# tambetm/simple_dqn

Hardware: NVIDIA B200
Metric: DQN training steps/sec (batch 32, 84x84x4) (higher is better)
Workload: dtype f16x3-split (fp32 accumulate)

## Files before the change

### simple_dqn_b200/csrc/net.cu

```cuda
#include <stdlib.h>

#include <new>
#include <vector>

#include <cuda_fp16.h>

#include "net.cuh"
#include "net_umma.cuh"

namespace b200 {

struct HeadTrainArgs {
  int enable;
  const uint8_t* actions;
  const int64_t* rewards;
  const uint8_t* terminals;
  const int32_t* midx;
  double discount;
  int min_reward, max_reward;
  float clip;
  float* delta;
  const uint32_t* step;
  float* row_cost;
  float* dz4;
// ... 655 lines not shown
    B2_CHECK_CUDA(cudaEventRecord(ev[11], sB));
    B2_CHECK_CUDA(cudaEventRecord(ev[12], sC));
    B2_CHECK_CUDA(cudaStreamWaitEvent(st, ev[11], 0));
    B2_CHECK_CUDA(cudaStreamWaitEvent(st, ev[12], 0));
  }
  B2_CHECK_CUDA(cudaEventRecord(ev[4], sA));
  B2_CHECK_CUDA(cudaStreamWaitEvent(st, ev[4], 0));
  return B200DQN_OK;
}

static int backward_and_update(b200dqn_net* n, const FrameSource& fs, int rows, cudaStream_t st, bool update) {
  if (update && n->world > 1 && !g_prof_on && n->use_branches && st != nullptr &&
      n->cfg.math_mode == B200DQN_MATH_TCGEN05)
    return backward_and_update_multi(n, fs, rows, st);
  const bool branches = update && n->world == 1 && n->use_branches && (st != nullptr || g_prof_on);
  if (!branches) {
    for (int op = kFc1Wgrad; op <= kConv1Wgrad; ++op) B2_TRY(bwd_op(n, fs, rows, BwdOp(op), st));
    B2_TRY(cost_finish_on(n, rows, st));
    if (!update) return B200DQN_OK;
    if (n->world > 1) {
      B2_TRY(optimizer_range(n, 0, kLayers - 1, 1 | 2, rows, st, "grad_reduce"));
      B2_TRY(comm_allreduce_grads(n, st));
      B2_PROF("allreduce", st);
      B2_TRY(optimizer_range(n, 0, kLayers - 1, 4, rows, st, "optimizer"));
    } else {
      B2_TRY(optimizer_range(n, 0, kLayers - 1, 1 | 4, rows, st, "optimizer"));
    }
    return B200DQN_OK;
  }
  cudaStream_t sA = g_prof_on ? st : n->side[0], sB = g_prof_on ? st : n->side[1], sC = g_prof_on ? st : n->side[2];
  cudaStream_t sN = g_prof_on ? st : n->side[3];
  cudaEvent_t* ev = n->ev;
  const bool tc = n->cfg.math_mode == B200DQN_MATH_TCGEN05;
  static const bool fc1_fused_epilogue = getenv("B200DQN_FC1_FUSED") != nullptr;
  static const int nopdl_ops = getenv("B200DQN_NOPDL_OPS") ? int(strtol(getenv("B200DQN_NOPDL_OPS"), nullptr, 0)) : 0;
  if (getenv("B200DQN_WGRAD_ONE_STREAM") && !g_prof_on) sC = sB;
  auto chain_op = [&](BwdOp op) -> int {
    if (nopdl_ops >> int(op) & 1) {
      NoPdlScope plain;
      return bwd_op(n, fs, rows, op, st);
    }
    return bwd_op(n, fs, rows, op, st);
  };
  B2_CHECK_CUDA(cudaEventRecord(ev[0], st));
  B2_CHECK_CUDA(cudaStreamWaitEvent(sA, ev[0], 0));
  B2_CHECK_CUDA(cudaStreamWaitEvent(sN, ev[0], 0));
  {
    NoPdlScope side;
    if (!(tc && fc1_fused_epilogue)) B2_TRY(bwd_op(n, fs, rows, kFc1Wgrad, sA));
    B2_TRY(cost_finish_on(n, rows, sN));
    if (tc) B2_TRY(opt_fc2_small(n, rows, sN));
  }
  B2_TRY(chain_op(kFc1Dgrad));
  B2_CHECK_CUDA(cudaEventRecord(ev[1], st));
  static const char* fc1_when_env = getenv("B200DQN_OPT_FC1_WHEN");
  const int fc1_when = !fc1_when_env || g_prof_on ? 0 : !strcmp(fc1_when_env, "ev2") ? 2 : !strcmp(fc1_when_env, "ev3") ? 3
                       : !strcmp(fc1_when_env, "last") ? 4 : !strcmp(fc1_when_env, "skip") ? 5 : 0;
  auto opt_fc1_now = [&]() -> int {
    NoPdlScope side;
    if (tc && fc1_fused_epilogue) return umma_fc1_wgrad_fused(n, rows, sA, n->keep_grads);
    if (tc && n->defer_fc1) return fc1_update_deferred(n, sA);
    if (tc) return umma_opt_fc1(n, rows, sA);
    return optimizer_range(n, 3, 4, 1 | 4, rows, sA, "opt_fc");
  };
  B2_CHECK_CUDA(cudaStreamWaitEvent(sA, ev[1], 0));
  if (fc1_when == 0) B2_TRY(opt_fc1_now());
  B2_CHECK_CUDA(cudaStreamWaitEvent(sB, ev[1], 0));
  { NoPdlScope side; B2_TRY(bwd_op(n, fs, rows, kConv3Wgrad, sB)); }
  B2_TRY(chain_op(kConv3Dgrad));
  B2_CHECK_CUDA(cudaEventRecord(ev[2], st));
  if (fc1_when == 2) {
    B2_CHECK_CUDA(cudaStreamWaitEvent(sA, ev[2], 0));
    B2_TRY(opt_fc1_now());
  }
  B2_CHECK_CUDA(cudaStreamWaitEvent(sB, ev[2], 0));
  {
    NoPdlScope side;
    if (n->cfg.math_mode == B200DQN_MATH_TCGEN05) B2_TRY(umma_opt_conv(n, 2, rows, sB, "opt_conv3"));
    else B2_TRY(optimizer_range(n, 2, 2, 1 | 4, rows, sB, "opt_conv3"));
  }
  B2_CHECK_CUDA(cudaStreamWaitEvent(sC, ev[2], 0));
  { NoPdlScope side; B2_TRY(bwd_op(n, fs, rows, kConv2Wgrad, sC)); }
  B2_TRY(chain_op(kConv2Dgrad));
  B2_CHECK_CUDA(cudaEventRecord(ev[3], st));
  if (fc1_when == 3) {
    B2_CHECK_CUDA(cudaStreamWaitEvent(sA, ev[3], 0));
    B2_TRY(opt_fc1_now());
  }
  B2_CHECK_CUDA(cudaStreamWaitEvent(sC, ev[3], 0));
  {
    NoPdlScope side;
    if (n->cfg.math_mode == B200DQN_MATH_TCGEN05) B2_TRY(umma_opt_conv(n, 1, rows, sC, "opt_conv2"));
    else B2_TRY(optimizer_range(n, 1, 1, 1 | 4, rows, sC, "opt_conv2"));
  }
  B2_TRY(chain_op(kConv1Wgrad));
// ... 645 lines not shown

extern "C" int b200dqn_net_device_ptr(b200dqn_net* n, int which, void** dev_ptr, size_t* bytes) {
  B2_REQUIRE(n && dev_ptr, B200DQN_EINVAL, "net_device_ptr: null argument");
  void* p = nullptr;
  size_t b = 0;
  switch (which) {
    case B200DQN_NET_PTR_Q_ONLINE: p = n->d_q[0]; b = size_t(n->nb) * n->A * 4; break;
    case B200DQN_NET_PTR_Q_TARGET: p = n->d_q[1]; b = size_t(n->nb) * n->A * 4; break;
    case B200DQN_NET_PTR_DELTAS: p = n->d_delta; b = size_t(n->nb) * n->A * 4; break;
    case B200DQN_NET_PTR_GRADS: p = n->d_g; b = n->n_params * 4; break;
    case B200DQN_NET_PTR_WEIGHTS: p = n->d_w; b = n->n_params * 4; break;
    case B200DQN_NET_PTR_COST: p = n->d_cost; b = kCostRing * 4; break;
    case B200DQN_NET_PTR_H1: p = n->d_h1[0]; b = size_t(n->nb) * kP1 * kP1 * kC1 * 4; break;
    case B200DQN_NET_PTR_H2: p = n->d_h2[0]; b = size_t(n->nb) * kP2 * kP2 * kC2 * 4; break;
    case B200DQN_NET_PTR_H3: p = n->d_h3[0]; b = size_t(n->nb) * kFlat * 4; break;
    case B200DQN_NET_PTR_H4: p = n->d_h4[0]; b = size_t(n->nb) * kHidden * 4; break;
    default: B2_REQUIRE(false, B200DQN_EINVAL, "net_device_ptr: unknown selector %d", which);
  }
  *dev_ptr = p;
  if (bytes) *bytes = b;
  return B200DQN_OK;
}

extern "C" int b200dqn_net_set_keep_grads(b200dqn_net* n, int keep) {
  B2_REQUIRE(n, B200DQN_EINVAL, "null net");
  n->keep_grads = keep != 0;
  destroy_step_graphs(n);
  if (n->graph_train_exec) { cudaGraphExecDestroy(n->graph_train_exec); n->graph_train_exec = nullptr; }
  return B200DQN_OK;
}

extern "C" int b200dqn_net_get_grads(b200dqn_net* n, int layer, float* host_dW, void* stream) {
  B2_REQUIRE(n && host_dW && layer >= 0 && layer < kLayers, B200DQN_EINVAL, "net_get_grads: bad argument");
  B2_REQUIRE(n->cfg.math_mode != B200DQN_MATH_TCGEN05 || n->world > 1 || n->keep_grads ||
                 getenv("B200DQN_FC1_FUSED") == nullptr,
             B200DQN_ESTATE, "net_get_grads: call b200dqn_net_set_keep_grads(net, 1) before the step (fused optimizer)");
  DeviceGuard g(n->device);
  cudaStream_t st = as_stream(stream);
  const int64_t n4 = n->n_params / 4;
  if (n->world == 1) {
    k_optimizer<<<cdiv(n4, 256), 256, 0, st>>>(n->lt, n->d_part, n->d_g, n->d_w, n->d_s, 0, n4, 1 | 2, OptArgs{},
                                               KTrace{nullptr, 0});
    B2_LAUNCH_CHECK();
  } else if (n->xchg_ok && n->xchg_sched == 2 && n->d_xbuf && layer == 3) {
    const int64_t b4 = n->lt.off[3] / 4, e4 = n->lt.off[4] / 4;
    k_optimizer<<<cdiv(e4 - b4, 256), 256, 0, st>>>(n->lt, n->d_part, n->d_g, n->d_w, n->d_s, b4, e4, 1 | 2, OptArgs{},
                                                    KTrace{nullptr, 0});
    B2_LAUNCH_CHECK();
  }
  return xfer_params(n, n->d_g, layer, host_dW, false, st);
}

extern "C" int b200dqn_net_launches_per_step(const b200dqn_net* n, int* launches) {
  B2_REQUIRE(n && launches, B200DQN_EINVAL, "null argument");
  if (n->graph_def_launches > 0) {
    *launches = n->graph_def_launches;
  } else if (n->graph_launches > 0) {
    *launches = n->graph_launches;
  } else {
    const bool tc = n->cfg.math_mode == B200DQN_MATH_TCGEN05;
    *launches = 1 + 4 + 1 + 7 + (n->world > 1 ? (tc ? 7 : 2) : (tc ? 6 : 4));
  }
  return B200DQN_OK;
}
```

### simple_dqn_b200/csrc/net_umma.cu

```cuda
#include "net.cuh"
#include "net_umma.cuh"
#include "umma.cuh"
#include "umma2.cuh"
#include "umma_mn.cuh"
#include "conv1_tma.cuh"

namespace b200 {

__device__ __forceinline__ void ld8(const float* p, float v[8]) {
  const float4 a = *reinterpret_cast<const float4*>(p);
  const float4 b = *reinterpret_cast<const float4*>(p + 4);
  v[0] = a.x; v[1] = a.y; v[2] = a.z; v[3] = a.w; v[4] = b.x; v[5] = b.y; v[6] = b.z; v[7] = b.w;
}
__device__ __forceinline__ void st8(float* p, const float v[8]) {
  *reinterpret_cast<float4*>(p) = make_float4(v[0], v[1], v[2], v[3]);
  *reinterpret_cast<float4*>(p + 4) = make_float4(v[4], v[5], v[6], v[7]);
}
__device__ __forceinline__ void zero8(float v[8]) {
#pragma unroll
  for (int i = 0; i < 8; ++i) v[i] = 0.f;
}

struct UmmaState {
  __half* h16[3][2] = {};
  int64_t h_elems[3] = {};
  __half* dz16[4] = {};
  int64_t dz_elems[4] = {};
  uint8_t* img_fwd[2][4] = {};
  int64_t img_fwd_bytes[4] = {};
  uint8_t* im2col1 = nullptr;
  uint8_t* img_dgr[3] = {};
};
static inline UmmaState* ust(b200dqn_net* n) { return static_cast<UmmaState*>(n->umma_state); }

struct PlanePair {
  __half* hi;
  int64_t lo_off;
};
// ... 187 lines not shown
    return {(int64_t(n * P + yy) * P + xx) * KO, yy, xx, ok};
  }
  __device__ bool a_chunk(int, const umma2::RowCtx& rc, int kk, int64_t& off) const {
    const int rp = kk / (RT * KO), sp = (kk / KO) % RT, ko = kk % KO;
    const int p = rc.y - rp, q = rc.x - sp;
    off = rc.base - (rp * P + sp) * KO + ko;
    return p >= 0 && p < P && q >= 0 && q < P;
  }
  __device__ const uint8_t* b_tile(int z, int, int kb) const { return wimg + (int64_t(z) * (K / 64) + kb) * (C * 256); }
  __device__ void prefetch8(int z, int m, int c0, float pf[8]) const {
    const int n = m / (HC * HC), yx = m % (HC * HC), yy = yx / HC, xx = yx % HC;
    const int y = yy * ST + z / ST, xq = xx * ST + z % ST;
    if (y >= H || xq >= H) { zero8(pf); return; }
    ld8(x + (int64_t(n * H + y) * H + xq) * C + c0, pf);
  }
  __device__ void store8p(int z, int m, int c0, const float v[8], const float xv[8]) const {
    const int n = m / (HC * HC), yx = m % (HC * HC), yy = yx / HC, xx = yx % HC;
    const int y = yy * ST + z / ST, xq = xx * ST + z % ST;
    if (y >= H || xq >= H) return;
    const int64_t i = (int64_t(n * H + y) * H + xq) * C + c0;
    float o[8];
#pragma unroll
    for (int j = 0; j < 8; ++j) o[j] = xv[j] > 0.f ? v[j] : 0.f;
    if (dx) st8(dx + i, o);
    if (dx16.hi) umma2::split8_planes(o, dx16.hi + i, dx16.hi + dx16.lo_off + i);
  }
};

template <int H, int C, int R, int ST, int KO, int STG = 4>
struct WConvWgrad {
  static constexpr int P = (H - R) / ST + 1, KW = R * R * C;
  static_assert((R * C) % 64 == 0 && KO == 64, "64-element runs must not straddle a filter row");
  static constexpr int kBN = 64, kStages = STG;
  static constexpr bool kAExact = false, kARegs = false, kABulk = false, kFusedUpdate = false;
  PlanePair x16;
  PlanePair dz16;
  float* part;
  int rows, kb_per_split;
  __device__ int M(int) const { return KW; }
  __device__ int N(int) const { return KO; }
  __device__ void krange(int z, int& kb, int& ke) const {
    const int total = (rows * P * P + 63) / 64;
    kb = min(z * kb_per_split, total);
    ke = min(kb + kb_per_split, total);
  }
  __device__ umma_mn::PixCtx pix(int, int kpix) const {
    const int n = kpix / (P * P), pq = kpix % (P * P);
    return {n, pq / P, pq % P, kpix < rows * P * P};
  }
  __device__ umma2::Planes a_planes(int) const { return {x16.hi, x16.lo_off}; }
  __device__ bool a_run(int, const umma_mn::PixCtx& px, int mchunk, int64_t& off) const {
    const int m = mchunk * 64, r = m / (R * C), sc = m % (R * C);
    off = (int64_t(px.n * H + px.p * ST + r) * H + px.q * ST) * C + sc;
    return m < KW;
  }
  __device__ umma2::Planes b_planes(int) const { return {dz16.hi, dz16.lo_off}; }
  __device__ int64_t b_off(int, const umma_mn::PixCtx& px) const { return (int64_t(px.n * P + px.p) * P + px.q) * KO; }
  __device__ void store8(int z, int m, int n0, const float v[8]) const { st8(part + (int64_t(z) * KW + m) * KO + n0, v); }
};

struct WConv1Wgrad {
  static constexpr int kBN = 32, kStages = 4;
  static constexpr bool kAExact = true, kARegs = false, kABulk = true, kFusedUpdate = false;
  const uint8_t* im2col;
  PlanePair dz16;
  float* part;
  int rows, kb_per_split;
  int tile_rows;
  __device__ int M(int) const { return kK1; }
  __device__ int N(int) const { return kC1; }
  __device__ int total_kb() const {
    return tile_rows == 128 ? (rows * kP1 * kP1 + 63) / 64 : rows * conv1tma::kTilesPerSample * 2;
  }
  __device__ void krange(int z, int& kb, int& ke) const {
    const int total = total_kb();
    kb = min(z * kb_per_split, total);
    ke = min(kb + kb_per_split, total);
  }
  __device__ umma_mn::PixCtx pix(int, int kpix) const {
    if (tile_rows == 128) return {kpix, 0, 0, kpix < rows * kP1 * kP1};
    const int tile = kpix >> 7, local = kpix & 127;
    return {tile * tile_rows + local, 0, 0, local < tile_rows && tile < rows * conv1tma::kTilesPerSample};
  }
  __device__ const uint8_t* a_sub(int, int c, int kb) const {
    return im2col + (int64_t(kb >> 1) * (kK1 / 64) + c) * (128 * 128) + (kb & 1) * (64 * 128);
  }
  __device__ umma2::Planes b_planes(int) const { return {dz16.hi, dz16.lo_off}; }
  __device__ int64_t b_off(int, const umma_mn::PixCtx& px) const { return int64_t(px.n) * kC1; }
  __device__ void store8(int z, int m, int n0, const float v[8]) const {
    float o[8];
#pragma unroll
    for (int j = 0; j < 8; ++j) o[j] = v[j] * (1.0f / 255.0f);
    st8(part + (int64_t(z) * kK1 + m) * kC1 + n0, o);
  }
};

struct WFc1Wgrad {
  static constexpr int kBN = 64, kStages = 2;
  static constexpr bool kAExact = false, kARegs = false, kABulk = false, kFusedUpdate = false;
  PlanePair h3_16;
  PlanePair dz4_16;
  float* dw4;
  int rows;
  __device__ int M(int) const { return kFlat; }
  __device__ int N(int) const { return kHidden; }
  __device__ void krange(int, int& kb, int& ke) const { kb = 0; ke = (rows + 63) / 64; }
  __device__ umma_mn::PixCtx pix(int, int b) const { return {b, 0, 0, b < rows}; }
  __device__ umma2::Planes a_planes(int) const { return {h3_16.hi, h3_16.lo_off}; }
  __device__ bool a_run(int, const umma_mn::PixCtx& px, int mchunk, int64_t& off) const {
    off = int64_t(px.n) * kFlat + mchunk * 64;
    return mchunk * 64 < kFlat;
  }
  __device__ umma2::Planes b_planes(int) const { return {dz4_16.hi, dz4_16.lo_off}; }
  __device__ int64_t b_off(int, const umma_mn::PixCtx& px) const { return int64_t(px.n) * kHidden; }
  __device__ void store8(int, int m, int n0, const float v[8]) const { st8(dw4 + int64_t(m) * kHidden + n0, v); }
};

struct WFc1WgradGather {
  static constexpr int kBN = 64, kStages = 2;
  static constexpr bool kAExact = false, kARegs = false, kABulk = false, kFusedUpdate = false;
  const __half* h3g;
  const __half* dzg;
  int64_t h3_parity, h3_lo, dz_parity, dz_lo;
  const uint32_t* epoch;
  float* dw4;
  int rows;
  __device__ int M(int) const { return kFlat; }
  __device__ int N(int) const { return kHidden; }
  __device__ void krange(int, int& kb, int& ke) const { kb = 0; ke = (rows + 63) / 64; }
  __device__ umma_mn::PixCtx pix(int, int b) const { return {b, 0, 0, b < rows}; }
  __device__ umma2::Planes a_planes(int) const { return {h3g + int64_t(epoch[0] & 1) * h3_parity, h3_lo}; }
  __device__ bool a_run(int, const umma_mn::PixCtx& px, int mchunk, int64_t& off) const {
    off = int64_t(px.n) * kFlat + mchunk * 64;
    return mchunk * 64 < kFlat;
  }
  __device__ umma2::Planes b_planes(int) const { return {dzg + int64_t(epoch[1] & 1) * dz_parity, dz_lo}; }
  __device__ int64_t b_off(int, const umma_mn::PixCtx& px) const { return int64_t(px.n) * kHidden; }
  __device__ void store8(int, int m, int n0, const float v[8]) const { st8(dw4 + int64_t(m) * kHidden + n0, v); }
};

struct WFc1WgradFused {
  static constexpr int kBN = 64, kStages = 2;
  static constexpr bool kAExact = false, kARegs = false, kABulk = false, kFusedUpdate = true;
  PlanePair h3_16;
  PlanePair dz4_16;
  float* w;
  float* s;
  float* dw_out;
  uint8_t* img_dgr;
  int rows;
  OptArgs opt;
  __device__ int M(int) const { return kFlat; }
  __device__ int N(int) const { return kHidden; }
  __device__ void krange(int, int& kb, int& ke) const { kb = 0; ke = (rows + 63) / 64; }
  __device__ umma_mn::PixCtx pix(int, int b) const { return {b, 0, 0, b < rows}; }
  __device__ umma2::Planes a_planes(int) const { return {h3_16.hi, h3_16.lo_off}; }
  __device__ bool a_run(int, const umma_mn::PixCtx& px, int mchunk, int64_t& off) const {
    off = int64_t(px.n) * kFlat + mchunk * 64;
    return mchunk * 64 < kFlat;
  }
  __device__ umma2::Planes b_planes(int) const { return {dz4_16.hi, dz4_16.lo_off}; }
  __device__ int64_t b_off(int, const umma_mn::PixCtx& px) const { return int64_t(px.n) * kHidden; }
  __device__ void store8(int, int, int, const float*) const {}
  __device__ float step_scalar() const { return opt_step_scalar(opt); }
  __device__ void update8(int, int m, int n0, float l, const float g[8], float nw[8]) const {
    const int64_t i = int64_t(m) * kHidden + n0;
    if (dw_out) st8(dw_out + i, g);
    opt_update_vec<8>(opt, l, g, nw, w + i, s + i);
    uint4 hi, lo;
    umma::split8(nw, hi, lo);
    uint8_t* base = img_dgr + (int64_t(m / 128) * (kHidden / 64) + n0 / 64) * (128 * 256) +
                    umma::sw128_off(m % 128, (n0 % 64) / 8);
    *reinterpret_cast<uint4*>(base) = hi;
    *reinterpret_cast<uint4*>(base + 128 * 128) = lo;
  }
  __device__ void pack_col8(int, int, int, const float*) const {}
};

template <int K, int N>
struct PackFwdConv {
  static constexpr bool kRowMajorThreads = false;
  const float* w;
  __host__ __device__ int tiles() const { return 1; }
  __host__ __device__ int rows() const { return N; }
  __host__ __device__ int kblocks() const { return K / 64; }
  __device__ void src8(int, int r, int k0, float v[8]) const {
#pragma unroll
    for (int j = 0; j < 8; ++j) v[j] = w[(k0 + j) * N + r];
  }
};
struct PackFc1Dgrad {
  static constexpr bool kRowMajorThreads = true;
  const float* w;
  __host__ __device__ int tiles() const { return (kFlat + 127) / 128; }
  __host__ __device__ int rows() const { return 128; }
  __host__ __device__ int kblocks() const { return kHidden / 64; }
  __device__ void src8(int tile, int r, int k0, float v[8]) const {
    const int m = tile * 128 + r;
    if (m >= kFlat) { zero8(v); return; }
    ld8(w + m * kHidden + k0, v);
  }
};
template <int H, int C, int R, int ST, int KO>
struct PackConvDgrad {
  static constexpr int RT = R / ST, K = RT * RT * KO;
  static constexpr bool kRowMajorThreads = true;
  const float* w;
  __host__ __device__ int tiles() const { return ST * ST; }
  __host__ __device__ int rows() const { return C; }
// ... 477 lines not shown
      using P2 = WConvWgrad<kP1, kC1, 4, 2, kC2, 2>;
      if (shallow_ring(n, "conv2_wgrad")) {
        P2 p{PlanePair{u->h16[0][0], u->h_elems[0]}, PlanePair{u->dz16[2], u->dz_elems[2]},
             n->d_part + lt.part_off[1], rows, umma_wgrad_kb(1, rows)};
        return umma_mn::launch_umma_mn("conv2_wgrad", p, P::KW, kC2, lt.splits[1], st);
      }
      P p{PlanePair{u->h16[0][0], u->h_elems[0]}, PlanePair{u->dz16[2], u->dz_elems[2]},
          n->d_part + lt.part_off[1], rows, umma_wgrad_kb(1, rows)};
      return umma_mn::launch_umma_mn("conv2_wgrad", p, P::KW, kC2, lt.splits[1], st);
    }
    case 5: {
      UmmaState* u = ust(n);
      using P = V2ConvDgrad<kP1, kC1, 4, 2, kC2>;
      using P2 = V2ConvDgrad<kP1, kC1, 4, 2, kC2, 2>;
      if (shallow_ring(n, "conv2_dgrad")) {
        P2 p{PlanePair{u->dz16[2], u->dz_elems[2]}, u->img_dgr[2], n->d_h1[0], n->keep_grads ? n->d_dz1 : nullptr,
             PlanePair{u->dz16[3], u->dz_elems[3]}, rows};
        return umma2::launch_umma2("conv2_dgrad", p, rows * P::HC * P::HC, kC1, 4, st);
      }
      P p{PlanePair{u->dz16[2], u->dz_elems[2]}, u->img_dgr[2], n->d_h1[0], n->keep_grads ? n->d_dz1 : nullptr,
          PlanePair{u->dz16[3], u->dz_elems[3]}, rows};
      return umma2::launch_umma2("conv2_dgrad", p, rows * P::HC * P::HC, kC1, 4, st);
    }
    default: {
      UmmaState* u = ust(n);
      (void)src; (void)idx; (void)shift;
      WConv1Wgrad p{u->im2col1, PlanePair{u->dz16[3], u->dz_elems[3]}, n->d_part + lt.part_off[0], rows,
                    umma_wgrad_kb(0, rows), g_conv1_tma ? conv1tma::kTileRows : 128};
      return umma_mn::launch_umma_mn("conv1_wgrad", p, kK1, kC1, lt.splits[0], st);
    }
  }
}

int umma_fc1_wgrad_fused(b200dqn_net* n, int rows, cudaStream_t st, bool keep_grads) {
  UmmaState* u = ust(n);
  const LayerTable& lt = n->lt;
  WFc1WgradFused p{PlanePair{u->h16[2][0], u->h_elems[2]}, PlanePair{u->dz16[0], u->dz_elems[0]},
                   n->d_w + lt.off[3], n->d_s + lt.off[3], keep_grads ? n->d_part + lt.part_off[3] : nullptr,
                   u->img_dgr[0], rows, make_opt_args(n, rows)};
  return umma_mn::launch_umma_mn("fc1_wgrad+opt", p, kFlat, kHidden, 1, st);
}

int umma_fc1_splits(int rows) { return fc1_splits_for(rows); }
bool umma_has_backward() { return true; }
int umma_push_h3(b200dqn_net* n, cudaStream_t st) {
  UmmaState* u = ust(n);
  cudaStream_t sN = n->side[3];
  B2_CHECK_CUDA(cudaEventRecord(n->ev[13], st));
  B2_CHECK_CUDA(cudaStreamWaitEvent(sN, n->ev[13], 0));
  const int rc = comm_push_planes(n, 0, u->h16[2][0], u->h_elems[2], sN);
  if (rc) return rc;
  B2_CHECK_CUDA(cudaEventRecord(n->ev[14], sN));
  return B200DQN_OK;
}
int umma_push_dz4(b200dqn_net* n, cudaStream_t st) {
  UmmaState* u = ust(n);
  return comm_push_planes(n, 1, u->dz16[0], u->dz_elems[0], st);
}
int umma_gather_dz4_ll(b200dqn_net* n, cudaStream_t st) {
  UmmaState* u = ust(n);
  return comm_gather_dz4_ll(n, u->dz16[0], u->dz_elems[0], st, true);
}
int umma_fc1_wgrad_gathered(b200dqn_net* n, cudaStream_t st) {
  WFc1WgradGather p{reinterpret_cast<const __half*>(n->d_xbuf + n->x_h3_off),
                    reinterpret_cast<const __half*>(n->d_xbuf + n->x_dz_off),
                    n->x_h3_parity / 2, n->x_h3_lo, n->x_dz_parity / 2, n->x_dz_lo,
                    n->d_xpush_epoch, n->d_part + n->lt.part_off[3], n->nb * n->world};
  return umma_mn::launch_umma_mn("fc1_wgrad", p, kFlat, kHidden, 1, st);
}

int umma_forward_launches() { return 4; }
int umma_backward_launches() { return 7; }

// ... 7 lines not shown
```

### simple_dqn_b200/csrc/net_umma.cuh

```cuda
#pragma once
#include <cuda_fp16.h>

#include "common.cuh"
#include "comm_p2p.cuh"
#include "optim.cuh"

struct b200dqn_net;

namespace b200 {

OptArgs make_opt_args(const b200dqn_net* n, int rows);

int umma_net_init(b200dqn_net* n);
void umma_net_destroy(b200dqn_net* n);
int umma_weights_changed(b200dqn_net* n, cudaStream_t st);
int umma_target_synced(b200dqn_net* n, cudaStream_t st);
int umma_forward(b200dqn_net* n, const uint8_t* const src[2], const int32_t* const idx[2], const int shift[2],
                 const int64_t nframes[2], int nets, int rows, cudaStream_t st);
int umma_fc1_splits(int rows);
int umma_opt_fc1(b200dqn_net* n, int rows, cudaStream_t st, bool from_g = false, const uint32_t* gate = nullptr);
int umma_fc1_wgrad_fused(b200dqn_net* n, int rows, cudaStream_t st, bool keep_grads);
int umma_opt_conv(b200dqn_net* n, int l, int rows, cudaStream_t st, const char* label, bool from_g = false);
int umma_pack_layers(b200dqn_net* n, int which, int l0, int l1, cudaStream_t st);
void umma_dz4_planes(b200dqn_net* n, __half** hi, int64_t* lo_off);
int umma_wgrad_splits(int layer, int rows);
bool umma_has_backward();
int umma_backward_op(b200dqn_net* n, int op, const uint8_t* src, const int32_t* idx, int shift, int rows,
                     cudaStream_t st);
int umma_forward_launches();
int umma_backward_launches();

int comm_allreduce_grads(b200dqn_net* n, cudaStream_t st);
int comm_allreduce_range(b200dqn_net* n, int l0, int l1, cudaStream_t st);
int comm_xchg_range(b200dqn_net* n, int l0, int l1, int chan, cudaStream_t st, const char* label);
bool comm_gather_active(const b200dqn_net* n, cudaStream_t st);
int comm_xll_layer(b200dqn_net* n, int layer, cudaStream_t st, const char* label);
int comm_xll_args(b200dqn_net* n, int layer, XllArgs* out);
int umma_opt_conv_xll(b200dqn_net* n, int l, int rows, cudaStream_t st, const char* label);
int comm_push_planes(b200dqn_net* n, int chan, const void* hi, int64_t lo_off_elems, cudaStream_t st);
int comm_wait_pushes(b200dqn_net* n, cudaStream_t st, int dz_rows = 0);
bool comm_dz4_ll_enabled();
int comm_gather_dz4_ll(b200dqn_net* n, const void* hi, int64_t lo_off_elems, cudaStream_t st, bool wait_h3);
bool comm_head_push(const b200dqn_net* n, cudaStream_t st, HeadPush* out);
int umma_push_h3(b200dqn_net* n, cudaStream_t st);
int umma_push_dz4(b200dqn_net* n, cudaStream_t st);
int umma_gather_dz4_ll(b200dqn_net* n, cudaStream_t st);
int umma_fc1_wgrad_gathered(b200dqn_net* n, cudaStream_t st);
void comm_destroy(b200dqn_net* n);

}
```

### simple_dqn_b200/csrc/umma_mn.cuh

```cuda
#pragma once
#include "umma2.cuh"

namespace b200 {
namespace umma_mn {

using umma::kBM;
using umma2::kLoadThreads;
using umma2::kThreads2;
using umma2::Planes;

constexpr int kKB = 64;

using umma::make_desc_mn;
__host__ __device__ constexpr uint32_t make_idesc_f16_mn(int M, int N) {
  return (1u << 4) | (1u << 15) | (1u << 16) | (uint32_t(N >> 3) << 17) | (uint32_t(M >> 4) << 24);
}
__device__ __forceinline__ uint32_t mn_off(int kr, int j) {
  return uint32_t((kr >> 3) * 1024 + (kr & 7) * 128 + ((j ^ (kr & 7)) << 4));
}

struct PixCtx {
  int n, p, q;
  bool ok;
};
// ... 146 lines not shown
          umma2::cp_async16(dst + mn_off(kr, 4 + sub), src + bpl.lo_off + sub * 8, bytes);
        }
      }
      if constexpr (P::kARegs) fence_proxy_async_smem();
      umma2::cp_async_arrive_noinc(&s_full[s]);
    }

    pdl_launch_dependents();

    mbar_wait(&s_done, 0);
    umma::fence_after_sync();
    {
      const int q = warp & 3, half = warp >> 2;
      const int row = q * 32 + lane;
      const uint32_t lane_addr = tmem + (uint32_t(q * 32) << 16);
      constexpr int kColsPerHalf = BN / 2;
      constexpr int kChunks = kColsPerHalf / 8;
      constexpr int kPitch = BN * 4 + 16;
#pragma unroll
      for (int c = 0; c < kChunks; ++c) {
        const int col = half * kColsPerHalf + c * 8;
        float a0[8], a1[8];
        umma::tmem_ld8(lane_addr + col, a0);
        umma::tmem_ld8(lane_addr + BN + col, a1);
        umma::tmem_ld_wait();
#pragma unroll
        for (int j = 0; j < 8; ++j) a0[j] = fmaf(a1[j], umma::kLoInv, a0[j]);
        float* dst = reinterpret_cast<float*>(smem_gen + row * kPitch + col * 4);
        *reinterpret_cast<float4*>(dst) = make_float4(a0[0], a0[1], a0[2], a0[3]);
        *reinterpret_cast<float4*>(dst + 4) = make_float4(a0[4], a0[5], a0[6], a0[7]);
      }
      umma2::named_bar_sync(1, kLoadThreads);
      constexpr int kChunksPerRow = BN / 8;
      if constexpr (!P::kFusedUpdate) {
#pragma unroll
        for (int i = 0; i < kBM * kChunksPerRow / kLoadThreads; ++i) {
          const int id = tid + i * kLoadThreads;
          const int r = id / kChunksPerRow, cc = id % kChunksPerRow;
          const float* src = reinterpret_cast<const float*>(smem_gen + r * kPitch + cc * 32);
          const float4 v0 = *reinterpret_cast<const float4*>(src), v1 = *reinterpret_cast<const float4*>(src + 4);
          const float v[8] = {v0.x, v0.y, v0.z, v0.w, v1.x, v1.y, v1.z, v1.w};
          if (m0 + r < M && n0 + cc * 8 < N) p.store8(z, m0 + r, n0 + cc * 8, v);
        }
      } else {
        constexpr int kIt = kBM * kChunksPerRow / kLoadThreads;
        const float l_step = p.step_scalar();
#pragma unroll
        for (int i = 0; i < kIt; ++i) {
          const int id = tid + i * kLoadThreads;
          const int r = id / kChunksPerRow, cc = id % kChunksPerRow;
          float* src = reinterpret_cast<float*>(smem_gen + r * kPitch + cc * 32);
          const float4 v0 = *reinterpret_cast<const float4*>(src), v1 = *reinterpret_cast<const float4*>(src + 4);
          const float g[8] = {v0.x, v0.y, v0.z, v0.w, v1.x, v1.y, v1.z, v1.w};
          if (m0 + r < M && n0 + cc * 8 < N) {
            float nw[8];
            p.update8(z, m0 + r, n0 + cc * 8, l_step, g, nw);
            *reinterpret_cast<float4*>(src) = make_float4(nw[0], nw[1], nw[2], nw[3]);
            *reinterpret_cast<float4*>(src + 4) = make_float4(nw[4], nw[5], nw[6], nw[7]);
          }
        }
        umma2::named_bar_sync(1, kLoadThreads);
#pragma unroll
        for (int i = 0; i < (kBM / 8) * BN / kLoadThreads; ++i) {
          const int id = tid + i * kLoadThreads;
          const int nn = id % BN, mg = id / BN;
          if (m0 + mg * 8 < M && n0 + nn < N) {
            float wv[8];
#pragma unroll
            for (int j = 0; j < 8; ++j)
              wv[j] = *reinterpret_cast<const float*>(smem_gen + (mg * 8 + j) * kPitch + nn * 4);
            p.pack_col8(z, m0 + mg * 8, n0 + nn, wv);
          }
        }
      }
    }
  }
  umma::fence_before_sync();
  __syncthreads();
  if (warp == 8) {
    umma::fence_after_sync();
    umma::tmem_dealloc(tmem, C::kTmemCols);
  }
  kt_end(kt);
}

template <class P>
static int launch_umma_mn(const char* label, const P& p, int M, int N, int Z, cudaStream_t st) {
  using C = CfgMN<P>;
  static bool configured = false;
  if (!configured) {
    B2_CHECK_CUDA(cudaFuncSetAttribute(k_umma_mn<P>, cudaFuncAttributeMaxDynamicSharedMemorySize, C::kSmemBytes));
    configured = true;
  }
  dim3 grid((M + kBM - 1) / kBM, (N + C::BN - 1) / C::BN, Z);
  B2_CHECK_CUDA(launch_pdl(k_umma_mn<P>, grid, dim3(kThreads2), C::kSmemBytes, st, p, ktrace_slot(label)));
  B2_PROF(label, st);
  return B200DQN_OK;
}

}
}
```

Measured before the change: 13340.

## Add dedicated warp-specialized fc1 wgrad+Adam kernel with TMA weight/state streaming, enable by default

Adds a new persistent, warp-specialized kernel that computes the fc1 weight gradient with tcgen05 MMA into double-buffered TMEM accumulators. In the same kernel it applies the optimizer update, streaming weights and optimizer state through per-warp TMA load/store rings and writing the packed fp16 hi/lo swizzled image for the dgrad path. It becomes the default tc path whenever fc1 deferral is off, replacing the separate fc1 wgrad and fc1 optimizer launches and removing the old env-gated fused epilogue from the generic MN kernel. The aim is to cut one launch plus the round trip of the fp32 gradient through global memory, and to overlap MMA with the optimizer epilogue. The cost is a fixed CTA count (24 by default), host-side tensor-map encoding on every call, and more complex synchronization.

```diff
diff --git a/simple_dqn_b200/csrc/fc1_wgrad_opt.cuh b/simple_dqn_b200/csrc/fc1_wgrad_opt.cuh
--- /dev/null
+++ b/simple_dqn_b200/csrc/fc1_wgrad_opt.cuh
@@ -0,0 +1,228 @@
+#pragma once
+#include "conv1_tma.cuh"
+#include "optim.cuh"
+#include "umma_mn.cuh"
+
+namespace b200 {
+namespace fc1opt {
+
+constexpr int kUnitsM = (kFlat + 127) / 128;
+constexpr int kUnitsN = kHidden / 64;
+constexpr int kUnits = kUnitsM * kUnitsN;
+constexpr int kEpiWarps = 8;
+constexpr int kThreads = (kEpiWarps + 2) * 32;
+constexpr uint32_t kSub = 64 * 128;
+constexpr uint32_t kStageBytes = 6 * kSub;
+constexpr uint32_t kBox = 32 * 128;
+constexpr uint32_t kWarpRing = 4 * kBox;
+constexpr uint32_t kSmemBytes = 1024 + kStageBytes + kEpiWarps * kWarpRing;
+constexpr uint32_t kTmemCols = 256;
+constexpr uint32_t kImgTile = 128 * 256;
+
+__device__ __forceinline__ void tma_store_3d(const CUtensorMap* map, uint32_t smem_src, int c0, int c1, int c2) {
+  asm volatile("cp.async.bulk.tensor.3d.global.shared::cta.bulk_group [%0, {%2, %3, %4}], [%1];"
+               ::"l"(reinterpret_cast<uint64_t>(map)), "r"(smem_src), "r"(c0), "r"(c1), "r"(c2)
+               : "memory");
+}
+
+struct Params {
+  uint8_t* img;
+  float* dw_out;
+  int rows;
+  OptArgs opt;
+};
+
+__global__ void __launch_bounds__(kThreads, 1)
+k_fc1_wgrad_opt(const __grid_constant__ CUtensorMap h3_map, const __grid_constant__ CUtensorMap dz_map,
+                const __grid_constant__ CUtensorMap w_map, const __grid_constant__ CUtensorMap s_map, const Params p,
+                const KTrace kt) {
+  extern __shared__ uint8_t smem_raw[];
+  __shared__ uint32_t s_tmem;
+  __shared__ __align__(8) uint64_t s_op_full, s_op_empty;
+  __shared__ __align__(8) uint64_t s_acc_full[2], s_acc_empty[2];
+  __shared__ __align__(8) uint64_t s_ws_full[kEpiWarps][2];
+
+  const int tid = threadIdx.x, warp = tid >> 5, lane = tid & 31;
+  kt_begin(kt);
+  const int u0 = int(blockIdx.x) * kUnits / int(gridDim.x), u1 = (int(blockIdx.x) + 1) * kUnits / int(gridDim.x);
+  const int nunits = u1 - u0;
+  const int nkb = (p.rows + 63) / 64;
+  const int ns = p.opt.nstates;
+  const uint32_t slot_bytes = uint32_t(1 + ns) * kBox;
+  const int nslots = int(kWarpRing / slot_bytes);
+
+  const uint32_t smem_base = (smem_u32(smem_raw) + 1023u) & ~1023u;
+  uint8_t* smem_gen = smem_raw + (smem_base - smem_u32(smem_raw));
+
+  if (warp == 8) umma::tmem_alloc(&s_tmem, kTmemCols);
+  if (tid == 32 * 9) {
+    mbar_init(&s_op_full, 1);
+    mbar_init(&s_op_empty, 1);
+    for (int b = 0; b < 2; ++b) {
+      mbar_init(&s_acc_full[b], 1);
+      mbar_init(&s_acc_empty[b], 4);
+    }
+    for (int w = 0; w < kEpiWarps; ++w)
+      for (int s = 0; s < 2; ++s) mbar_init(&s_ws_full[w][s], 1);
+    mbar_fence_init();
+    conv1tma::tma_prefetch_desc(&h3_map);
+    conv1tma::tma_prefetch_desc(&dz_map);
+  }
+  umma::fence_before_sync();
+  __syncthreads();
+  umma::fence_after_sync();
+  const uint32_t tmem = s_tmem;
+  pdl_wait();
+
+  if (warp < kEpiWarps) {
+    const int grp = warp >> 2, q = warp & 3;
+    const int my_units = (nunits - grp + 1) / 2;
+    const int nj = 2 * my_units;
+    const uint32_t ring = smem_base + kStageBytes + warp * kWarpRing;
+    uint8_t* ring_gen = smem_gen + kStageBytes + warp * kWarpRing;
+    auto coords = [&](int j, int& u, int& row0, int& col0) {
+      u = u0 + grp + 2 * (j >> 1);
+      row0 = (u / kUnitsN) * 128 + q * 32;
+      col0 = (u % kUnitsN) * 64 + (j & 1) * 32;
+    };
+    auto fetch = [&](int j) {
+      int u, row0, col0;
+      coords(j, u, row0, col0);
+      const int s = j % nslots;
+      const uint32_t dst = ring + s * slot_bytes;
+      mbar_arrive_expect_tx(&s_ws_full[warp][s], slot_bytes);
+      conv1tma::tma_load_3d(dst, &w_map, col0, row0, 0, &s_ws_full[warp][s]);
+      conv1tma::tma_load_3d(dst + kBox, &s_map, col0, row0, 0, &s_ws_full[warp][s]);
+    };
+    if (lane == 0)
+      for (int j = 0; j < nj && j < nslots; ++j) fetch(j);
+
+    OptArgs os = p.opt;
+    os.plane = kBox / 4;
+    const float l_step = opt_step_scalar(p.opt);
+    const int r = q * 32 + lane;
+    const uint32_t tbase = tmem + (uint32_t(q * 32) << 16) + uint32_t(grp * 128);
+    for (int j = 0; j < nj; ++j) {
+      int u, row0, col0;
+      coords(j, u, row0, col0);
+      const int h = j & 1, li = grp + 2 * (j >> 1);
+      if (h == 0) {
+        mbar_wait(&s_acc_full[grp], uint32_t(li >> 1) & 1u);
+        umma::fence_after_sync();
+      }
+      float g[32];
+#pragma unroll
+      for (int c = 0; c < 4; ++c) {
+        float a0[8], a1[8];
+        umma::tmem_ld8(tbase + h * 32 + c * 8, a0);
+        umma::tmem_ld8(tbase + 64 + h * 32 + c * 8, a1);
+        umma::tmem_ld_wait();
+#pragma unroll
+        for (int e = 0; e < 8; ++e) g[c * 8 + e] = fmaf(a1[e], umma::kLoInv, a0[e]);
+      }
+      if (h == 1) {
+        umma::fence_before_sync();
+        __syncwarp();
+        if (lane == 0) mbar_arrive(&s_acc_empty[grp]);
+      }
+      const int s = j % nslots;
+      mbar_wait(&s_ws_full[warp][s], uint32_t(j / nslots) & 1u);
+      uint8_t* slot = ring_gen + s * slot_bytes;
+      const int m = row0 + lane;
+      uint8_t* img = p.img + int64_t(u) * kImgTile;
+#pragma unroll
+      for (int c = 0; c < 4; ++c) {
+        float nw[8];
+#pragma unroll
+        for (int e = 0; e < 2; ++e) {
+          const uint32_t off = uint32_t(lane) * 128 + ((uint32_t(2 * c + e) ^ uint32_t(lane & 7)) << 4);
+          opt_update_vec<4>(os, l_step, g + c * 8 + e * 4, nw + e * 4, reinterpret_cast<float*>(slot + off),
+                            reinterpret_cast<float*>(slot + kBox + off));
+        }
+        if (m < kFlat) {
+          uint4 hi, lo;
+          umma::split8(nw, hi, lo);
+          uint8_t* dst = img + umma::sw128_off(r, h * 4 + c);
+          *reinterpret_cast<uint4*>(dst) = hi;
+          *reinterpret_cast<uint4*>(dst + 128 * 128) = lo;
+          if (p.dw_out) {
+            float* gd = p.dw_out + int64_t(m) * kHidden + col0 + c * 8;
+            *reinterpret_cast<float4*>(gd) = make_float4(g[c * 8], g[c * 8 + 1], g[c * 8 + 2], g[c * 8 + 3]);
+            *reinterpret_cast<float4*>(gd + 4) = make_float4(g[c * 8 + 4], g[c * 8 + 5], g[c * 8 + 6], g[c * 8 + 7]);
+          }
+        }
+      }
+      fence_proxy_async_smem();
+      __syncwarp();
+      if (lane == 0) {
+        const uint32_t src = ring + s * slot_bytes;
+        tma_store_3d(&w_map, src, col0, row0, 0);
+        tma_store_3d(&s_map, src + kBox, col0, row0, 0);
+        tma_bulk_commit();
+        if (j + nslots < nj) {
+          tma_bulk_wait_read_all();
+          fetch(j + nslots);
+        }
+      }
+      __syncwarp();
+    }
+    if (lane == 0) tma_bulk_wait_all();
+  } else if (warp == 8) {
+    constexpr uint32_t idesc_full = umma_mn::make_idesc_f16_mn(128, 128);
+    constexpr uint32_t idesc_hi = umma_mn::make_idesc_f16_mn(128, 64);
+    const uint64_t da_hi = umma::make_desc_mn(smem_base, kSub);
+    const uint64_t da_lo = umma::make_desc_mn(smem_base + 2 * kSub, kSub);
+    const uint64_t db = umma::make_desc_mn(smem_base + 4 * kSub, kSub);
+    int it = 0;
+    for (int li = 0; li < nunits; ++li) {
+      const int b = li & 1;
+      if (li >= 2) {
+        mbar_wait(&s_acc_empty[b], uint32_t((li >> 1) - 1) & 1u);
+        umma::fence_after_sync();
+      }
+      const uint32_t d = tmem + uint32_t(b * 128);
+      for (int kb = 0; kb < nkb; ++kb, ++it) {
+        mbar_wait(&s_op_full, uint32_t(it) & 1u);
+        umma::fence_after_sync();
+        if (umma2::elect_one()) {
+#pragma unroll
+          for (int k = 0; k < 4; ++k) {
+            umma::mma_f16(d, da_hi + 128 * k, db + 128 * k, idesc_full, (kb > 0 || k > 0) ? 1u : 0u);
+            umma::mma_f16(d + 64, da_lo + 128 * k, db + 128 * k, idesc_hi, 1u);
+          }
+          umma::mma_commit(&s_op_empty);
+          if (kb == nkb - 1) umma::mma_commit(&s_acc_full[b]);
+        }
+        __syncwarp();
+      }
+    }
+  } else {
+    int it = 0, prev_mb = -1;
+    for (int li = 0; li < nunits && lane == 0; ++li) {
+      const int u = u0 + li, mb = u / kUnitsN, nt = u % kUnitsN;
+      for (int kb = 0; kb < nkb; ++kb, ++it) {
+        if (it > 0) mbar_wait(&s_op_empty, uint32_t(it - 1) & 1u);
+        const bool keep_a = nkb == 1 && mb == prev_mb;
+        mbar_arrive_expect_tx(&s_op_full, keep_a ? 2 * kSub : kStageBytes);
+        if (!keep_a)
+          for (int pl = 0; pl < 2; ++pl)
+            for (int c = 0; c < 2; ++c)
+              conv1tma::tma_load_3d(smem_base + (pl * 2 + c) * kSub, &h3_map, mb * 128 + c * 64, kb * 64, pl, &s_op_full);
+        for (int pl = 0; pl < 2; ++pl)
+          conv1tma::tma_load_3d(smem_base + (4 + pl) * kSub, &dz_map, nt * 64, kb * 64, pl, &s_op_full);
+      }
+      prev_mb = mb;
+    }
+    __syncwarp();
+  }
+  umma::fence_before_sync();
+  __syncthreads();
+  if (warp == 8) {
+    umma::fence_after_sync();
+    umma::tmem_dealloc(tmem, kTmemCols);
+  }
+  kt_end(kt);
+}
+
+}
+}
diff --git a/simple_dqn_b200/csrc/net.cu b/simple_dqn_b200/csrc/net.cu
--- a/simple_dqn_b200/csrc/net.cu
+++ b/simple_dqn_b200/csrc/net.cu
@@ -711,7 +711,7 @@
   cudaStream_t sN = g_prof_on ? st : n->side[3];
   cudaEvent_t* ev = n->ev;
   const bool tc = n->cfg.math_mode == B200DQN_MATH_TCGEN05;
-  static const bool fc1_fused_epilogue = getenv("B200DQN_FC1_FUSED") != nullptr;
+  const bool fc1_one_kernel = tc && !n->defer_fc1;
   static const int nopdl_ops = getenv("B200DQN_NOPDL_OPS") ? int(strtol(getenv("B200DQN_NOPDL_OPS"), nullptr, 0)) : 0;
   if (getenv("B200DQN_WGRAD_ONE_STREAM") && !g_prof_on) sC = sB;
   auto chain_op = [&](BwdOp op) -> int {
@@ -726,7 +726,7 @@
   B2_CHECK_CUDA(cudaStreamWaitEvent(sN, ev[0], 0));
   {
     NoPdlScope side;
-    if (!(tc && fc1_fused_epilogue)) B2_TRY(bwd_op(n, fs, rows, kFc1Wgrad, sA));
+    if (!fc1_one_kernel) B2_TRY(bwd_op(n, fs, rows, kFc1Wgrad, sA));
     B2_TRY(cost_finish_on(n, rows, sN));
     if (tc) B2_TRY(opt_fc2_small(n, rows, sN));
   }
@@ -737,9 +737,8 @@
                        : !strcmp(fc1_when_env, "last") ? 4 : !strcmp(fc1_when_env, "skip") ? 5 : 0;
   auto opt_fc1_now = [&]() -> int {
     NoPdlScope side;
-    if (tc && fc1_fused_epilogue) return umma_fc1_wgrad_fused(n, rows, sA, n->keep_grads);
-    if (tc && n->defer_fc1) return fc1_update_deferred(n, sA);
-    if (tc) return umma_opt_fc1(n, rows, sA);
+    if (fc1_one_kernel) return umma_fc1_wgrad_opt(n, rows, sA);
+    if (tc) return fc1_update_deferred(n, sA);
     return optimizer_range(n, 3, 4, 1 | 4, rows, sA, "opt_fc");
   };
   B2_CHECK_CUDA(cudaStreamWaitEvent(sA, ev[1], 0));
@@ -1451,9 +1450,8 @@
 
 extern "C" int b200dqn_net_get_grads(b200dqn_net* n, int layer, float* host_dW, void* stream) {
   B2_REQUIRE(n && host_dW && layer >= 0 && layer < kLayers, B200DQN_EINVAL, "net_get_grads: bad argument");
-  B2_REQUIRE(n->cfg.math_mode != B200DQN_MATH_TCGEN05 || n->world > 1 || n->keep_grads ||
-                 getenv("B200DQN_FC1_FUSED") == nullptr,
-             B200DQN_ESTATE, "net_get_grads: call b200dqn_net_set_keep_grads(net, 1) before the step (fused optimizer)");
+  B2_REQUIRE(n->cfg.math_mode != B200DQN_MATH_TCGEN05 || n->world > 1 || n->keep_grads, B200DQN_ESTATE,
+             "net_get_grads: call b200dqn_net_set_keep_grads(net, 1) before the step (fused fc1 update)");
   DeviceGuard g(n->device);
   cudaStream_t st = as_stream(stream);
   const int64_t n4 = n->n_params / 4;
@@ -1478,7 +1476,7 @@
     *launches = n->graph_launches;
   } else {
     const bool tc = n->cfg.math_mode == B200DQN_MATH_TCGEN05;
-    *launches = 1 + 4 + 1 + 7 + (n->world > 1 ? (tc ? 7 : 2) : (tc ? 6 : 4));
-  }
-  return B200DQN_OK;
-}
+    *launches = 1 + 4 + 1 + 7 + (n->world > 1 ? (tc ? 7 : 2) : (tc ? 5 : 4));
+  }
+  return B200DQN_OK;
+}
diff --git a/simple_dqn_b200/csrc/net_umma.cu b/simple_dqn_b200/csrc/net_umma.cu
--- a/simple_dqn_b200/csrc/net_umma.cu
+++ b/simple_dqn_b200/csrc/net_umma.cu
@@ -4,6 +4,7 @@
 #include "umma2.cuh"
 #include "umma_mn.cuh"
 #include "conv1_tma.cuh"
+#include "fc1_wgrad_opt.cuh"
 
 namespace b200 {
 
@@ -257,7 +258,7 @@
   static constexpr int P = (H - R) / ST + 1, KW = R * R * C;
   static_assert((R * C) % 64 == 0 && KO == 64, "64-element runs must not straddle a filter row");
   static constexpr int kBN = 64, kStages = STG;
-  static constexpr bool kAExact = false, kARegs = false, kABulk = false, kFusedUpdate = false;
+  static constexpr bool kAExact = false, kARegs = false, kABulk = false;
   PlanePair x16;
   PlanePair dz16;
   float* part;
@@ -286,7 +287,7 @@
 
 struct WConv1Wgrad {
   static constexpr int kBN = 32, kStages = 4;
-  static constexpr bool kAExact = true, kARegs = false, kABulk = true, kFusedUpdate = false;
+  static constexpr bool kAExact = true, kARegs = false, kABulk = true;
   const uint8_t* im2col;
   PlanePair dz16;
   float* part;
@@ -322,7 +323,7 @@
 
 struct WFc1Wgrad {
   static constexpr int kBN = 64, kStages = 2;
-  static constexpr bool kAExact = false, kARegs = false, kABulk = false, kFusedUpdate = false;
+  static constexpr bool kAExact = false, kARegs = false, kABulk = false;
   PlanePair h3_16;
   PlanePair dz4_16;
   float* dw4;
@@ -343,7 +344,7 @@
 
 struct WFc1WgradGather {
   static constexpr int kBN = 64, kStages = 2;
-  static constexpr bool kAExact = false, kARegs = false, kABulk = false, kFusedUpdate = false;
+  static constexpr bool kAExact = false, kARegs = false, kABulk = false;
   const __half* h3g;
   const __half* dzg;
   int64_t h3_parity, h3_lo, dz_parity, dz_lo;
@@ -362,44 +363,6 @@
   __device__ umma2::Planes b_planes(int) const { return {dzg + int64_t(epoch[1] & 1) * dz_parity, dz_lo}; }
   __device__ int64_t b_off(int, const umma_mn::PixCtx& px) const { return int64_t(px.n) * kHidden; }
   __device__ void store8(int, int m, int n0, const float v[8]) const { st8(dw4 + int64_t(m) * kHidden + n0, v); }
-};
-
-struct WFc1WgradFused {
-  static constexpr int kBN = 64, kStages = 2;
-  static constexpr bool kAExact = false, kARegs = false, kABulk = false, kFusedUpdate = true;
-  PlanePair h3_16;
-  PlanePair dz4_16;
-  float* w;
-  float* s;
-  float* dw_out;
-  uint8_t* img_dgr;
-  int rows;
-  OptArgs opt;
-  __device__ int M(int) const { return kFlat; }
-  __device__ int N(int) const { return kHidden; }
-  __device__ void krange(int, int& kb, int& ke) const { kb = 0; ke = (rows + 63) / 64; }
-  __device__ umma_mn::PixCtx pix(int, int b) const { return {b, 0, 0, b < rows}; }
-  __device__ umma2::Planes a_planes(int) const { return {h3_16.hi, h3_16.lo_off}; }
-  __device__ bool a_run(int, const umma_mn::PixCtx& px, int mchunk, int64_t& off) const {
-    off = int64_t(px.n) * kFlat + mchunk * 64;
-    return mchunk * 64 < kFlat;
-  }
-  __device__ umma2::Planes b_planes(int) const { return {dz4_16.hi, dz4_16.lo_off}; }
-  __device__ int64_t b_off(int, const umma_mn::PixCtx& px) const { return int64_t(px.n) * kHidden; }
-  __device__ void store8(int, int, int, const float*) const {}
-  __device__ float step_scalar() const { return opt_step_scalar(opt); }
-  __device__ void update8(int, int m, int n0, float l, const float g[8], float nw[8]) const {
-    const int64_t i = int64_t(m) * kHidden + n0;
-    if (dw_out) st8(dw_out + i, g);
-    opt_update_vec<8>(opt, l, g, nw, w + i, s + i);
-    uint4 hi, lo;
-    umma::split8(nw, hi, lo);
-    uint8_t* base = img_dgr + (int64_t(m / 128) * (kHidden / 64) + n0 / 64) * (128 * 256) +
-                    umma::sw128_off(m % 128, (n0 % 64) / 8);
-    *reinterpret_cast<uint4*>(base) = hi;
-    *reinterpret_cast<uint4*>(base + 128 * 128) = lo;
-  }
-  __device__ void pack_col8(int, int, int, const float*) const {}
 };
 
 template <int K, int N>
@@ -943,13 +906,59 @@
   }
 }
 
-int umma_fc1_wgrad_fused(b200dqn_net* n, int rows, cudaStream_t st, bool keep_grads) {
+constexpr int kFc1OptCtas = 24;
+static int fc1_opt_ctas() {
+  const char* env = getenv("B200DQN_FC1_CTAS");
+  const int g = env ? atoi(env) : kFc1OptCtas;
+  return g < 1 ? 1 : g > fc1opt::kUnits ? fc1opt::kUnits : g;
+}
+
+static int make_map(CUtensorMap* map, CUtensorMapDataType type, const void* base, const cuuint64_t dims[3],
+                    const cuuint64_t strides[2], const cuuint32_t box[3]) {
+  conv1tma::EncodeTiledFn fn = conv1tma::encode_fn();
+  B2_REQUIRE(fn, B200DQN_ECUDA, "cuTensorMapEncodeTiled is not available from this driver");
+  B2_REQUIRE((reinterpret_cast<uintptr_t>(base) & 15) == 0 && strides[0] % 16 == 0 && strides[1] % 16 == 0,
+             B200DQN_EINVAL, "fc1_wgrad_opt: TMA needs 16-byte aligned bases and strides");
+  const cuuint32_t estr[3] = {1, 1, 1};
+  const CUresult r = fn(map, type, 3, const_cast<void*>(base), dims, strides, box, estr, CU_TENSOR_MAP_INTERLEAVE_NONE,
+                        CU_TENSOR_MAP_SWIZZLE_128B, CU_TENSOR_MAP_L2_PROMOTION_L2_256B, CU_TENSOR_MAP_FLOAT_OOB_FILL_NONE);
+  B2_REQUIRE(r == CUDA_SUCCESS, B200DQN_ECUDA, "cuTensorMapEncodeTiled failed (%d)", int(r));
+  return B200DQN_OK;
+}
+
+int umma_fc1_wgrad_opt(b200dqn_net* n, int rows, cudaStream_t st) {
   UmmaState* u = ust(n);
   const LayerTable& lt = n->lt;
-  WFc1WgradFused p{PlanePair{u->h16[2][0], u->h_elems[2]}, PlanePair{u->dz16[0], u->dz_elems[0]},
-                   n->d_w + lt.off[3], n->d_s + lt.off[3], keep_grads ? n->d_part + lt.part_off[3] : nullptr,
-                   u->img_dgr[0], rows, make_opt_args(n, rows)};
-  return umma_mn::launch_umma_mn("fc1_wgrad+opt", p, kFlat, kHidden, 1, st);
+  CUtensorMap h3m, dzm, wm, sm;
+  int rc;
+  {
+    const cuuint32_t box[3] = {64, 64, 1};
+    const cuuint64_t hd[3] = {cuuint64_t(kFlat), cuuint64_t(rows), 2};
+    const cuuint64_t hs[2] = {cuuint64_t(kFlat) * 2, cuuint64_t(u->h_elems[2]) * 2};
+    if ((rc = make_map(&h3m, CU_TENSOR_MAP_DATA_TYPE_FLOAT16, u->h16[2][0], hd, hs, box))) return rc;
+    const cuuint64_t dd[3] = {cuuint64_t(kHidden), cuuint64_t(rows), 2};
+    const cuuint64_t ds[2] = {cuuint64_t(kHidden) * 2, cuuint64_t(u->dz_elems[0]) * 2};
+    if ((rc = make_map(&dzm, CU_TENSOR_MAP_DATA_TYPE_FLOAT16, u->dz16[0], dd, ds, box))) return rc;
+  }
+  {
+    const cuuint64_t wd[3] = {cuuint64_t(kHidden), cuuint64_t(kFlat), 1};
+    const cuuint64_t sd[3] = {cuuint64_t(kHidden), cuuint64_t(kFlat), cuuint64_t(n->n_states)};
+    const cuuint64_t ws[2] = {cuuint64_t(kHidden) * 4, cuuint64_t(n->n_params) * 4};
+    const cuuint32_t wbox[3] = {32, 32, 1}, sbox[3] = {32, 32, cuuint32_t(n->n_states)};
+    if ((rc = make_map(&wm, CU_TENSOR_MAP_DATA_TYPE_FLOAT32, n->d_w + lt.off[3], wd, ws, wbox))) return rc;
+    if ((rc = make_map(&sm, CU_TENSOR_MAP_DATA_TYPE_FLOAT32, n->d_s + lt.off[3], sd, ws, sbox))) return rc;
+  }
+  fc1opt::Params p{u->img_dgr[0], n->keep_grads ? n->d_part + lt.part_off[3] : nullptr, rows, make_opt_args(n, rows)};
+  static bool configured = false;
+  if (!configured) {
+    B2_CHECK_CUDA(cudaFuncSetAttribute(fc1opt::k_fc1_wgrad_opt, cudaFuncAttributeMaxDynamicSharedMemorySize,
+                                       int(fc1opt::kSmemBytes)));
+    configured = true;
+  }
+  B2_CHECK_CUDA(launch_pdl(fc1opt::k_fc1_wgrad_opt, dim3(fc1_opt_ctas()), dim3(fc1opt::kThreads), fc1opt::kSmemBytes, st,
+                           h3m, dzm, wm, sm, p, ktrace_slot("fc1_wgrad_opt")));
+  B2_PROF("fc1_wgrad_opt", st);
+  return B200DQN_OK;
 }
 
 int umma_fc1_splits(int rows) { return fc1_splits_for(rows); }
diff --git a/simple_dqn_b200/csrc/net_umma.cuh b/simple_dqn_b200/csrc/net_umma.cuh
--- a/simple_dqn_b200/csrc/net_umma.cuh
+++ b/simple_dqn_b200/csrc/net_umma.cuh
@@ -19,7 +19,7 @@
                  const int64_t nframes[2], int nets, int rows, cudaStream_t st);
 int umma_fc1_splits(int rows);
 int umma_opt_fc1(b200dqn_net* n, int rows, cudaStream_t st, bool from_g = false, const uint32_t* gate = nullptr);
-int umma_fc1_wgrad_fused(b200dqn_net* n, int rows, cudaStream_t st, bool keep_grads);
+int umma_fc1_wgrad_opt(b200dqn_net* n, int rows, cudaStream_t st);
 int umma_opt_conv(b200dqn_net* n, int l, int rows, cudaStream_t st, const char* label, bool from_g = false);
 int umma_pack_layers(b200dqn_net* n, int which, int l0, int l1, cudaStream_t st);
 void umma_dz4_planes(b200dqn_net* n, __half** hi, int64_t* lo_off);
diff --git a/simple_dqn_b200/csrc/umma_mn.cuh b/simple_dqn_b200/csrc/umma_mn.cuh
--- a/simple_dqn_b200/csrc/umma_mn.cuh
+++ b/simple_dqn_b200/csrc/umma_mn.cuh
@@ -202,46 +202,14 @@
       }
       umma2::named_bar_sync(1, kLoadThreads);
       constexpr int kChunksPerRow = BN / 8;
-      if constexpr (!P::kFusedUpdate) {
-#pragma unroll
-        for (int i = 0; i < kBM * kChunksPerRow / kLoadThreads; ++i) {
-          const int id = tid + i * kLoadThreads;
-          const int r = id / kChunksPerRow, cc = id % kChunksPerRow;
-          const float* src = reinterpret_cast<const float*>(smem_gen + r * kPitch + cc * 32);
-          const float4 v0 = *reinterpret_cast<const float4*>(src), v1 = *reinterpret_cast<const float4*>(src + 4);
-          const float v[8] = {v0.x, v0.y, v0.z, v0.w, v1.x, v1.y, v1.z, v1.w};
-          if (m0 + r < M && n0 + cc * 8 < N) p.store8(z, m0 + r, n0 + cc * 8, v);
-        }
-      } else {
-        constexpr int kIt = kBM * kChunksPerRow / kLoadThreads;
-        const float l_step = p.step_scalar();
-#pragma unroll
-        for (int i = 0; i < kIt; ++i) {
-          const int id = tid + i * kLoadThreads;
-          const int r = id / kChunksPerRow, cc = id % kChunksPerRow;
-          float* src = reinterpret_cast<float*>(smem_gen + r * kPitch + cc * 32);
-          const float4 v0 = *reinterpret_cast<const float4*>(src), v1 = *reinterpret_cast<const float4*>(src + 4);
-          const float g[8] = {v0.x, v0.y, v0.z, v0.w, v1.x, v1.y, v1.z, v1.w};
-          if (m0 + r < M && n0 + cc * 8 < N) {
-            float nw[8];
-            p.update8(z, m0 + r, n0 + cc * 8, l_step, g, nw);
-            *reinterpret_cast<float4*>(src) = make_float4(nw[0], nw[1], nw[2], nw[3]);
-            *reinterpret_cast<float4*>(src + 4) = make_float4(nw[4], nw[5], nw[6], nw[7]);
-          }
-        }
-        umma2::named_bar_sync(1, kLoadThreads);
-#pragma unroll
-        for (int i = 0; i < (kBM / 8) * BN / kLoadThreads; ++i) {
-          const int id = tid + i * kLoadThreads;
-          const int nn = id % BN, mg = id / BN;
-          if (m0 + mg * 8 < M && n0 + nn < N) {
-            float wv[8];
-#pragma unroll
-            for (int j = 0; j < 8; ++j)
-              wv[j] = *reinterpret_cast<const float*>(smem_gen + (mg * 8 + j) * kPitch + nn * 4);
-            p.pack_col8(z, m0 + mg * 8, n0 + nn, wv);
-          }
-        }
+#pragma unroll
+      for (int i = 0; i < kBM * kChunksPerRow / kLoadThreads; ++i) {
+        const int id = tid + i * kLoadThreads;
+        const int r = id / kChunksPerRow, cc = id % kChunksPerRow;
+        const float* src = reinterpret_cast<const float*>(smem_gen + r * kPitch + cc * 32);
+        const float4 v0 = *reinterpret_cast<const float4*>(src), v1 = *reinterpret_cast<const float4*>(src + 4);
+        const float v[8] = {v0.x, v0.y, v0.z, v0.w, v1.x, v1.y, v1.z, v1.w};
+        if (m0 + r < M && n0 + cc * 8 < N) p.store8(z, m0 + r, n0 + cc * 8, v);
       }
     }
   }
```

Result: slower. 5484, median of 6 (-58.9%).
